# SmoothKen/knn-svc

Hardware: AMD Instinct MI355X
Metric: audio-sec converted/sec (xRT) end-to-end, cold target pool (higher is better)
Workload: dtype f32; 1 GPU; north-star point per rank: 30 s source vs 10 min target pool (20 x 30 s), ckpt_type=mix, post_opt_0.2, cold (pool encoded inside the step); seeded random weights of WavLM-Large (6 layers executed) and the 22.9 M-param generator; nq=1500, np_per_rank=30000, wavlm_batch_chunks=32, pipeline_depth=2

## Files before the change

### knn_svc_amd/csrc/elementwise.hip

```cpp
#include "common.h"
#include <cstdlib>
#include "gemm2_core.h"

namespace {

__device__ __forceinline__ void store_split4(float* row, int c, f32x4 y) {
    g2_u32x2 hi, lo;
    f16x2_split4(y, KN_F16X2_A_SCALE, hi, lo);
    char* ob = (char*)row + (c >> 5) * 128 + (c & 31) * 2;
    *(g2_u32x2*)ob = hi;
    *(g2_u32x2*)(ob + 64) = lo;
}
__device__ __forceinline__ f32x4 load_split4(const float* row, int c) {
    const char* ib = (const char*)row + (c >> 5) * 128 + (c & 31) * 2;
    const g2_u32x2 hi = *(const g2_u32x2*)ib, lo = *(const g2_u32x2*)(ib + 64);
    f32x4 y;
#pragma unroll
    for (int e = 0; e < 4; ++e) {
        const unsigned short hb = (unsigned short)(hi[e >> 1] >> (16 * (e & 1))), lb = (unsigned short)(lo[e >> 1] >> (16 * (e & 1)));
        y[e] = ((float)__builtin_bit_cast(_Float16, hb) + (float)__builtin_bit_cast(_Float16, lb)) * (1.0f / KN_F16X2_A_SCALE);
    }
    return y;
}

__device__ __forceinline__ float gelu_erf(float v) {
#pragma clang fp contract(off)
    return kn_gelu(v);
}

template <int MAXV, int R>
__global__ __launch_bounds__(256) void layernorm_kernel(const float* __restrict__ x, long rows, int dim, int ldx,
                                                       const float* __restrict__ gamma, const float* __restrict__ beta,
                                                       int gelu, float* __restrict__ out, int ldo) {
#pragma clang fp contract(off)
    const int lane = threadIdx.x & 63;
    const long row0 = ((long)blockIdx.x * 4 + (threadIdx.x >> 6)) * R;
    if (row0 >= rows) return;
    f32x4 v[R][MAXV];
    float s[R];
#pragma unroll
    for (int r = 0; r < R; ++r) {
        s[r] = 0.f;
        const bool ok = row0 + r < rows;
        const float* xr = x + (row0 + r) * (long)ldx;
#pragma unroll
        for (int i = 0; i < MAXV; ++i) {
            const int c = lane * 4 + 256 * i;
            if (ok && c < dim) { v[r][i] = *(const f32x4*)(xr + c); s[r] += (v[r][i][0] + v[r][i][1]) + (v[r][i][2] + v[r][i][3]); }
            else v[r][i] = (f32x4){0.f, 0.f, 0.f, 0.f};
        }
    }
    float mean[R], q[R];
#pragma unroll
    for (int r = 0; r < R; ++r) mean[r] = wave_sum(s[r]) / (float)dim;
#pragma unroll
    for (int r = 0; r < R; ++r) {
        q[r] = 0.f;
#pragma unroll
        for (int i = 0; i < MAXV; ++i) {
            const int c = lane * 4 + 256 * i;
            if (c < dim) {
#pragma unroll
                for (int e = 0; e < 4; ++e) { const float d = v[r][i][e] - mean[r]; q[r] = fmaf(d, d, q[r]); }
            }
        }
    }
#pragma unroll
    for (int r = 0; r < R; ++r) {
        const float var = wave_sum(q[r]) / (float)dim;
        const float rstd = 1.0f / sqrtf(var + 1e-5f);
        if (row0 + r >= rows) continue;
        float* orow = out + (row0 + r) * (long)ldo;
#pragma unroll
        for (int i = 0; i < MAXV; ++i) {
            const int c = lane * 4 + 256 * i;
            if (c < dim) {
                const f32x4 g = *(const f32x4*)(gamma + c), b = *(const f32x4*)(beta + c);
                f32x4 y;
#pragma unroll
                for (int e = 0; e < 4; ++e) {
                    float t = fmaf((v[r][i][e] - mean[r]) * rstd, g[e], b[e]);
                    y[e] = (gelu & 1) ? gelu_erf(t) : t;
                }
                if (gelu & 2) store_split4(orow, c, y);
                else *(f32x4*)(orow + c) = y;
            }
        }
    }
}

template <int CPL, int KMAXT, int RP>
__global__ __launch_bounds__(256) void conv0_ln_gelu_kernel(const float* __restrict__ x, long L, long T, int k, int stride,
                                                           const float* __restrict__ w, const float* __restrict__ gamma,
                                                           const float* __restrict__ beta, float* __restrict__ out, int split, int subs) {
    __shared__ float xs[2][64 * 8 + 32];
    const int lane = threadIdx.x & 63, wave = threadIdx.x >> 6;
    const int C = CPL * 64;
    const long b = blockIdx.y;
    const float* xb = x + b * L;
    const int span = 63 * stride + k;
    constexpr int NP = (CPL + 1) / 2;
    f32x2 wr[NP][KMAXT], g[NP], be[NP];
#pragma unroll
    for (int c = 0; c < NP; ++c) {
        const int ch = lane * CPL + 2 * c, ch1 = CPL > 1 ? ch + 1 : ch;
        g[c] = (f32x2){gamma[ch], gamma[ch1]}; be[c] = (f32x2){beta[ch], beta[ch1]};
#pragma unroll
        for (int t = 0; t < KMAXT; ++t) wr[c][t] = t < k ? (f32x2){w[ch * k + t], w[ch1 * k + t]} : (f32x2){0.f, 0.f};
    }
  for (int sub = 0; sub < subs; ++sub) {
    const long m0 = ((long)blockIdx.x * subs + sub) * 64;
    if (m0 >= T) break;
    float* xsb = xs[sub & 1];
    for (int i = threadIdx.x; i < span; i += 256) {
        const long p = m0 * stride + i;
        xsb[i] = p < L ? xb[p] : 0.f;
    }
    __syncthreads();
    for (int r = 0; r < 16; r += RP) {
        f32x2 y[RP][NP];
        float s[RP], mean[RP], q[RP], rstd[RP];
#pragma unroll
        for (int u = 0; u < RP; ++u) {
            const int lm = wave * 16 + r + u;
            float xv[KMAXT];
#pragma unroll
            for (int t = 0; t < KMAXT; ++t) xv[t] = t < k ? xsb[lm * stride + t] : 0.f;
            s[u] = 0.f;
#pragma unroll
            for (int c = 0; c < NP; ++c) {
                f32x2 a = {0.f, 0.f};
#pragma unroll
                for (int t = 0; t < KMAXT; ++t) a = __builtin_elementwise_fma(wr[c][t], (f32x2)(xv[t]), a);
                y[u][c] = a; s[u] += a[0]; if (CPL > 1) s[u] += a[1];
            }
        }
#pragma unroll
        for (int u = 0; u < RP; ++u) mean[u] = (RP > 1 ? wave_sum_dpp(s[u]) : wave_sum(s[u])) / (float)C;
#pragma unroll
        for (int u = 0; u < RP; ++u) {
            q[u] = 0.f;
#pragma unroll
            for (int c = 0; c < CPL; ++c) { const float d = y[u][c >> 1][c & 1] - mean[u]; q[u] += d * d; }
        }
#pragma unroll
        for (int u = 0; u < RP; ++u) rstd[u] = 1.0f / sqrtf((RP > 1 ? wave_sum_dpp(q[u]) : wave_sum(q[u])) / (float)C + 1e-5f);
#pragma unroll
        for (int u = 0; u < RP; ++u) {
            const long m = m0 + wave * 16 + r + u;
            if (m >= T) break;
            float* o = out + (b * T + m) * C + lane * CPL;
#pragma unroll
            for (int c = 0; c < NP; ++c) y[u][c] = kn_gelu2(__builtin_elementwise_fma((y[u][c] - mean[u]) * rstd[u], g[c], be[c]));
            if (CPL % 4 == 0) {
                if (split) {
                    float* orow = out + (b * T + m) * C;
#pragma unroll
                    for (int c = 0; c < CPL; c += 4) store_split4(orow, lane * CPL + c, (f32x4){y[u][c / 2][0], y[u][c / 2][1], y[u][c / 2 + 1][0], y[u][c / 2 + 1][1]});
                } else {
#pragma unroll
                    for (int c = 0; c < CPL; c += 4) *(f32x4*)(o + c) = (f32x4){y[u][c / 2][0], y[u][c / 2][1], y[u][c / 2 + 1][0], y[u][c / 2 + 1][1]};
                }
            } else {
#pragma unroll
                for (int c = 0; c < CPL; ++c) o[c] = y[u][c >> 1][c & 1];
            }
        }
    }
  }
}

__global__ __launch_bounds__(256) void gate_kernel(const float* __restrict__ xn, long rows, int heads, int ldx,
                                                  const float* __restrict__ w2, const float* __restrict__ b2,
                                                  const float* __restrict__ grep_a, float* __restrict__ gate, int split) {
    const int lane = threadIdx.x & 63;
    const long row = (long)blockIdx.x * 4 + (threadIdx.x >> 6);
    if (row >= rows) return;
    const int h = lane >> 2, part = lane & 3;
    float sa = 0.f, sb = 0.f;
    if (h < heads) {
        const float* xr = xn + row * (long)ldx + lane * 16;
#pragma unroll
        for (int e = 0; e < 16; e += 4) {
            const f32x4 xv = split ? load_split4(xn + row * (long)ldx, lane * 16 + e) : *(const f32x4*)(xr + e);
            const f32x4 wa = *(const f32x4*)(w2 + part * 16 + e), wb = *(const f32x4*)(w2 + 64 + part * 16 + e);
#pragma unroll
            for (int t = 0; t < 4; ++t) { sa += xv[t] * wa[t]; sb += xv[t] * wb[t]; }
        }
    }
    sa += __shfl_xor(sa, 1, 64); sa += __shfl_xor(sa, 2, 64);
    sb += __shfl_xor(sb, 1, 64); sb += __shfl_xor(sb, 2, 64);
    if (h < heads && part == 0) {
        const float ga = 1.0f / (1.0f + expf(-(sa + b2[0])));
        const float gb = 1.0f / (1.0f + expf(-(sb + b2[1])));
        gate[row * heads + h] = ga * (gb * grep_a[h] - 1.0f) + 2.0f;
    }
}

__global__ __launch_bounds__(256) void weighted_gather_kernel(const long* __restrict__ idx, const float* __restrict__ w,
                                                             long nq, int k, const float* __restrict__ pool, int dim,
                                                             int ld, float* __restrict__ out) {
#pragma clang fp contract(off)
    const long row = blockIdx.x;
    for (int c = threadIdx.x; c < dim; c += 256) {
        float acc = 0.f;
        for (int j = 0; j < k; ++j) {
            const float wj = w ? w[row * k + j] : 1.0f / (float)k;
            const float t = pool[idx[row * k + j] * (long)ld + c] * wj;
            acc = j == 0 ? t : acc + t;
        }
        out[row * (long)dim + c] = acc;
    }
}

__global__ void reflect_pad_kernel(const float* __restrict__ x, long n, int pad, float* __restrict__ out) {
    const long i = (long)blockIdx.x * blockDim.x + threadIdx.x;
    if (i >= n + 2 * (long)pad) return;
    long j = i - pad;
    if (j < 0) j = -j;
    if (j >= n) j = 2 * (n - 1) - j;
    out[i] = x[j];
}

__global__ void complex_mag_kernel(const float* __restrict__ reim, long rows, int bins, int ld, float* __restrict__ out) {
    const long i = (long)blockIdx.x * blockDim.x + threadIdx.x;
    if (i >= rows * bins) return;
    const long r = i / bins; const int b = (int)(i - r * bins);
    out[i] = hypotf(reim[r * ld + b], reim[r * ld + bins + b]);
}

__global__ void harmonic_amps_kernel(const float* __restrict__ spec, const float* __restrict__ f0, long T, int bins,
                                     int n_harm, float* __restrict__ harm) {
#pragma clang fp contract(off)
    const long i = (long)blockIdx.x * blockDim.x + threadIdx.x;
    if (i >= T * n_harm) return;
    const long t = i / n_harm; const int k = (int)(i - t * n_harm) + 1;
    const float f = f0[t];
    const float* s = spec + t * bins;
    float v;
    if (f == 0.f) {
        if (k == 1) { v = s[0]; for (int b = 1; b < bins; ++b) v = fmaxf(v, s[b]); }
        else v = 0.f;
    } else {
        const int nb = bins * 8;
        float pos = ((f * (float)k) * 2.0f) * (float)nb / 16000.0f;
        pos = fminf(pos, (float)nb);
        const int gi = (int)rintf(pos);
        if (gi >= nb) v = 0.f;
        else {
            float src = ((float)gi + 0.5f) * 0.125f - 0.5f;
            if (src < 0.f) src = 0.f;
            const int i0 = (int)src;
            const int i1 = i0 + (i0 < bins - 1 ? 1 : 0);
            const float l1 = src - (float)i0, l0 = 1.0f - l1;
            v = l0 * s[i0] + l1 * s[i1];
        }
    }
    harm[i] = 0.0108f * v;
}

__global__ __launch_bounds__(256) void reflect_pad_batch_kernel(const float* __restrict__ x, const long* __restrict__ offs, int pad,
                                                                float* __restrict__ out, long stride) {
    const int b = blockIdx.y;
    const long o0 = offs[b], n = offs[b + 1] - o0;
    float* ob = out + (long)b * stride;
    for (long i = (long)blockIdx.x * blockDim.x + threadIdx.x; i < stride; i += (long)gridDim.x * blockDim.x) {
        float v = 0.f;
        if (i < n + 2 * (long)pad) {
            long j = i - pad;
            if (j < 0) j = -j;
            if (j >= n) j = 2 * (n - 1) - j;
            v = x[o0 + j];
        }
        ob[i] = v;
    }
}

__global__ __launch_bounds__(256) void spec_harm_kernel(const float* __restrict__ reim, long rows, int bins, int ld,
                                                        const float* __restrict__ f0, int n_harm, float* __restrict__ spec,
                                                        float* __restrict__ harm) {
#pragma clang fp contract(off)
    extern __shared__ float sh[];
    const int wave = threadIdx.x >> 6, lane = threadIdx.x & 63;
    const long t = (long)blockIdx.x * 4 + wave;
    if (t >= rows) return;
    float* s = sh + wave * bins;
    const float* r = reim + t * (long)ld;
    float mx = 0.f;
    for (int b = lane; b < bins; b += 64) {
        const float v = hypotf(r[b], r[bins + b]);
        s[b] = v; spec[t * bins + b] = v;
        mx = fmaxf(mx, v);
    }
#pragma unroll
    for (int o = 32; o > 0; o >>= 1) mx = fmaxf(mx, __shfl_xor(mx, o, 64));
    const float f = f0[t];
    for (int k = lane + 1; k <= n_harm; k += 64) {
        float v;
        if (f == 0.f) v = k == 1 ? mx : 0.f;
        else {
            const int nb = bins * 8;
            float pos = ((f * (float)k) * 2.0f) * (float)nb / 16000.0f;
            pos = fminf(pos, (float)nb);
            const int gi = (int)rintf(pos);
            if (gi >= nb) v = 0.f;
            else {
                float src = ((float)gi + 0.5f) * 0.125f - 0.5f;
                if (src < 0.f) src = 0.f;
                const int i0 = (int)src;
                const int i1 = i0 + (i0 < bins - 1 ? 1 : 0);
                const float l1 = src - (float)i0, l0 = 1.0f - l1;
                v = l0 * s[i0] + l1 * s[i1];
            }
        }
        harm[t * n_harm + (k - 1)] = 0.0108f * v;
    }
}

__global__ __launch_bounds__(256) void mask_rows_kernel(float* __restrict__ x, int T, int dim, int ld, const int* __restrict__ lens) {
    const int b = blockIdx.y;
    const int len = lens[b];
    const long n4 = (long)(T - len) * (dim / 4);
    for (long i = (long)blockIdx.x * blockDim.x + threadIdx.x; i < n4; i += (long)gridDim.x * blockDim.x) {
        const long r = len + i / (dim / 4); const int c = (int)(i % (dim / 4)) * 4;
        *(f32x4*)(x + ((long)b * T + r) * ld + c) = (f32x4){0.f, 0.f, 0.f, 0.f};
    }
}

}

extern "C" int knnsvc_mask_rows(float* x, int32_t batches, int32_t T, int32_t dim, int32_t ld, const int32_t* lens, void* stream) {
    KN_REQUIRE(x && lens && batches > 0 && batches <= 65535 && T > 0 && dim > 0 && dim % 4 == 0 && ld >= dim && ld % 4 == 0 &&
               ((uintptr_t)x & 15) == 0, "mask_rows: bad arguments");
    hipLaunchKernelGGL(mask_rows_kernel, dim3(64, (unsigned)batches), dim3(256), 0, (hipStream_t)stream, x, T, dim, ld, lens);
    return knnsvc_check_launch("mask_rows");
}

extern "C" int knnsvc_layernorm(const float* x, int64_t rows, int32_t dim, int32_t ldx, const float* gamma,
                                const float* beta, int32_t gelu, float* out, int32_t ldo, void* stream) {
    KN_REQUIRE(x && gamma && beta && out, "layernorm: null pointer");
    KN_REQUIRE(dim > 0 && dim % 4 == 0 && dim <= 2048, "layernorm: dim must be a multiple of 4 and <= 2048");
    KN_REQUIRE(ldx % 4 == 0 && ldo % 4 == 0 && ldx >= dim && ldo >= dim, "layernorm: bad row strides");
    KN_REQUIRE(!(gelu & 2) || (dim % 32 == 0 && ldo % 32 == 0), "layernorm: split output needs dim % 32 == 0 and ldo % 32 == 0");
    KN_REQUIRE(((uintptr_t)x & 15) == 0 && ((uintptr_t)out & 15) == 0 && ((uintptr_t)gamma & 15) == 0 &&
               ((uintptr_t)beta & 15) == 0, "layernorm: pointers must be 16-byte aligned");
    if (rows <= 0) return KNNSVC_OK;
    hipStream_t st = (hipStream_t)stream;
    if (dim <= 512)
        hipLaunchKernelGGL((layernorm_kernel<2, 4>), dim3((unsigned)cdiv64(rows, 16)), dim3(256), 0, st, x, (long)rows, dim, ldx,
                           gamma, beta, gelu, out, ldo);
    else if (dim <= 1024)
        hipLaunchKernelGGL((layernorm_kernel<4, 2>), dim3((unsigned)cdiv64(rows, 8)), dim3(256), 0, st, x, (long)rows, dim, ldx,
                           gamma, beta, gelu, out, ldo);
    else
        hipLaunchKernelGGL((layernorm_kernel<8, 1>), dim3((unsigned)cdiv64(rows, 4)), dim3(256), 0, st, x, (long)rows, dim, ldx,
                           gamma, beta, gelu, out, ldo);
    return knnsvc_check_launch("layernorm");
}

extern "C" int knnsvc_wavlm_gate(const float* xn, int64_t rows, int32_t heads, int32_t head_dim, int32_t ldx,
                                 const float* w2, const float* b2, const float* grep_a, float* gate, int32_t x_f16x2, void* stream) {
    KN_REQUIRE(xn && w2 && b2 && grep_a && gate, "wavlm_gate: null pointer");
    KN_REQUIRE(head_dim == 64 && heads >= 1 && heads <= 16, "wavlm_gate: head_dim must be 64, heads <= 16");
    KN_REQUIRE(ldx % 4 == 0 && ldx >= heads * 64 && ((uintptr_t)xn & 15) == 0 && ((uintptr_t)w2 & 15) == 0,
               "wavlm_gate: alignment");
    if (rows <= 0) return KNNSVC_OK;
    hipLaunchKernelGGL(gate_kernel, dim3((unsigned)cdiv64(rows, 4)), dim3(256), 0, (hipStream_t)stream,
                       xn, (long)rows, heads, ldx, w2, b2, grep_a, gate, x_f16x2);
    return knnsvc_check_launch("wavlm_gate");
}

extern "C" int knnsvc_weighted_gather(const int64_t* idx, const float* w, int64_t nq, int32_t k, const float* pool,
                                      int32_t dim, int32_t ld, int32_t mean_mode, float* out, void* stream) {
    (void)mean_mode;
    KN_REQUIRE(idx && pool && out && k > 0 && dim > 0 && ld >= dim, "weighted_gather: bad arguments");
    KN_REQUIRE(w || (k & (k - 1)) == 0, "weighted_gather: uniform weights need a power-of-two k");
    if (nq <= 0) return KNNSVC_OK;
    hipLaunchKernelGGL(weighted_gather_kernel, dim3((unsigned)nq), dim3(256), 0, (hipStream_t)stream,
                       (const long*)idx, w, (long)nq, k, pool, dim, ld, out);
    return knnsvc_check_launch("weighted_gather");
}

extern "C" int knnsvc_reflect_pad(const float* x, int64_t n, int32_t pad, float* out, void* stream) {
    KN_REQUIRE(x && out && n > pad && pad >= 0, "reflect_pad: needs n > pad >= 0");
    const long tot = n + 2 * (long)pad;
    hipLaunchKernelGGL(reflect_pad_kernel, dim3((unsigned)cdiv64(tot, 256)), dim3(256), 0, (hipStream_t)stream,
                       x, (long)n, pad, out);
    return knnsvc_check_launch("reflect_pad");
}

extern "C" int knnsvc_reflect_pad_batch(const float* x, const int64_t* offs, int32_t batches, int32_t pad, float* out,
                                        int64_t stride, void* stream) {
    KN_REQUIRE(x && offs && out && batches > 0 && batches <= 65535 && pad >= 0 && stride > 2 * (int64_t)pad,
               "reflect_pad_batch: bad arguments (every item needs n > pad; stride > 2 pad)");
    const unsigned gx = (unsigned)(cdiv64(stride, 256) < 2048 ? cdiv64(stride, 256) : 2048);
    hipLaunchKernelGGL(reflect_pad_batch_kernel, dim3(gx, (unsigned)batches), dim3(256), 0, (hipStream_t)stream,
                       x, (const long*)offs, pad, out, (long)stride);
    return knnsvc_check_launch("reflect_pad_batch");
}

extern "C" int knnsvc_spec_harm(const float* reim, int64_t rows, int32_t bins, int32_t ld, const float* f0, int32_t n_harm,
                                float* spec, float* harm, void* stream) {
    KN_REQUIRE(reim && f0 && spec && harm && bins > 0 && bins <= 4096 && ld >= 2 * bins && n_harm > 0, "spec_harm: bad arguments");
    if (rows <= 0) return KNNSVC_OK;
    hipLaunchKernelGGL(spec_harm_kernel, dim3((unsigned)cdiv64(rows, 4)), dim3(256), (size_t)4 * bins * sizeof(float),
                       (hipStream_t)stream, reim, (long)rows, bins, ld, f0, n_harm, spec, harm);
    return knnsvc_check_launch("spec_harm");
}

extern "C" int knnsvc_complex_mag(const float* reim, int64_t rows, int32_t bins, int32_t ld, float* out, void* stream) {
    KN_REQUIRE(reim && out && bins > 0 && ld >= 2 * bins, "complex_mag: bad arguments");
    if (rows <= 0) return KNNSVC_OK;
    hipLaunchKernelGGL(complex_mag_kernel, dim3((unsigned)cdiv64(rows * bins, 256)), dim3(256), 0,
                       (hipStream_t)stream, reim, (long)rows, bins, ld, out);
    return knnsvc_check_launch("complex_mag");
}

extern "C" int knnsvc_harmonic_amps(const float* spec, const float* f0, int64_t T, int32_t bins, int32_t n_harm,
                                    float* harm, void* stream) {
    KN_REQUIRE(spec && f0 && harm && bins > 0 && n_harm > 0, "harmonic_amps: bad arguments");
    if (T <= 0) return KNNSVC_OK;
    hipLaunchKernelGGL(harmonic_amps_kernel, dim3((unsigned)cdiv64(T * n_harm, 256)), dim3(256), 0,
                       (hipStream_t)stream, spec, f0, (long)T, bins, n_harm, harm);
    return knnsvc_check_launch("harmonic_amps");
}

extern "C" int knnsvc_wavlm_conv0(const float* x, int32_t batches, int64_t L, const float* w, int32_t channels, int32_t k,
                                  int32_t stride, const float* gamma, const float* beta, float* out, int32_t out_f16x2, void* stream) {
    KN_REQUIRE(x && w && gamma && beta && out, "wavlm_conv0: null pointer");
    KN_REQUIRE(batches > 0 && batches <= 65535 && L >= k && k >= 1 && k <= 16 && stride >= 1 && stride <= 8,
               "wavlm_conv0: needs 1 <= k <= 16, 1 <= stride <= 8");
    KN_REQUIRE(channels == 64 || channels == 128 || channels == 256 || channels == 512, "wavlm_conv0: channels must be 64/128/256/512");
    KN_REQUIRE(!out_f16x2 || channels >= 256, "wavlm_conv0: split output needs >= 256 channels");
    const long T = (L - k) / stride + 1;
    hipStream_t st = (hipStream_t)stream;
    static int rp = -1, subs_env = -1;
    if (rp < 0) { const char* e = getenv("KNNSVC_CONV0_RP"); rp = e ? atoi(e) : 2; if (rp != 1 && rp != 4) rp = 2; }
    if (subs_env < 0) { const char* e = getenv("KNNSVC_CONV0_SUBS"); subs_env = e ? atoi(e) : 8; if (subs_env < 1 || subs_env > 64) subs_env = 8; }
    const int subs = cdiv64(T, 64L * subs_env) * batches >= 3072 ? subs_env : 1;
    dim3 grid((unsigned)cdiv64(T, 64L * subs), (unsigned)batches);
#define KN_C0R(CPL, KM, RP) hipLaunchKernelGGL((conv0_ln_gelu_kernel<CPL, KM, RP>), grid, dim3(256), 0, st, x, (long)L, T, k, stride, w, gamma, beta, out, out_f16x2, subs)
#define KN_C0(CPL, KM) { if (rp == 2) KN_C0R(CPL, KM, 2); else if (rp == 4) KN_C0R(CPL, KM, 4); else KN_C0R(CPL, KM, 1); }
    if (k <= 10) {
        if (channels == 512) KN_C0(8, 10) else if (channels == 256) KN_C0(4, 10) else if (channels == 128) KN_C0(2, 10) else KN_C0(1, 10)
    } else {
        if (channels == 512) KN_C0(8, 16) else if (channels == 256) KN_C0(4, 16) else if (channels == 128) KN_C0(2, 16) else KN_C0(1, 16)
    }
#undef KN_C0R
#undef KN_C0
    return knnsvc_check_launch("wavlm_conv0");
}

namespace {

__global__ __launch_bounds__(256) void round_f16_kernel(const float* __restrict__ x, long n, float* __restrict__ out) {
    const long i = ((long)blockIdx.x * 256 + threadIdx.x) * 4;
    if (i + 3 < n) {
        const f32x4 v = *(const f32x4*)(x + i);
        f32x4 r;
#pragma unroll
        for (int e = 0; e < 4; ++e) r[e] = (float)(_Float16)v[e];
        *(f32x4*)(out + i) = r;
    } else {
        for (long j = i; j < n; ++j) out[j] = (float)(_Float16)x[j];
    }
}

__global__ __launch_bounds__(256) void amp_ratio_kernel(const float* __restrict__ spec_q, int ld_q,
                                                       const float* __restrict__ spec_pool, int ld_pool, long np,
                                                       const long* __restrict__ idx, long nq, int k, int bins,
                                                       float* __restrict__ out) {
    const int lane = threadIdx.x & 63;
    const long t = (long)blockIdx.x * 4 + (threadIdx.x >> 6);
    if (t >= nq) return;
    double s = 0.0;
    for (int c = lane; c < bins; c += 64) s += (double)fabsf(spec_q[t * ld_q + c]);
    const float orig = (float)wave_sum_d(s);
    for (int j = 0; j < k; ++j) {
        long id = idx[t * k + j];
        id = id < 0 ? 0 : (id > np - 1 ? np - 1 : id);
        double a = 0.0;
        for (int c = lane; c < bins; c += 64) a += (double)fabsf(spec_pool[id * ld_pool + c]);
        const float l1 = (float)wave_sum_d(a);
        if (lane == 0) out[t * k + j] = orig / (l1 + 1e-5f);
    }
}

}

extern "C" int knnsvc_round_f16(const float* x, int64_t n, float* out, void* stream) {
    KN_REQUIRE(x && out && n >= 0, "round_f16: bad arguments");
    KN_REQUIRE(((uintptr_t)x & 15) == 0 && ((uintptr_t)out & 15) == 0, "round_f16: pointers must be 16-byte aligned");
    if (n == 0) return KNNSVC_OK;
    hipLaunchKernelGGL(round_f16_kernel, dim3((unsigned)cdiv64(n, 1024)), dim3(256), 0, (hipStream_t)stream, x, (long)n, out);
    return knnsvc_check_launch("round_f16");
}

extern "C" int knnsvc_amp_ratio(const float* spec_q, int32_t ld_q, const float* spec_pool, int32_t ld_pool, int64_t np,
                                const int64_t* idx, int64_t nq, int32_t k, int32_t bins, float* out, void* stream) {
    KN_REQUIRE(spec_q && spec_pool && idx && out, "amp_ratio: null pointer");
    KN_REQUIRE(np > 0 && k > 0 && bins > 0 && ld_q >= bins && ld_pool >= bins, "amp_ratio: bad sizes");
    if (nq <= 0) return KNNSVC_OK;
    hipLaunchKernelGGL(amp_ratio_kernel, dim3((unsigned)cdiv64(nq, 4)), dim3(256), 0, (hipStream_t)stream, spec_q, ld_q,
                       spec_pool, ld_pool, (long)np, (const long*)idx, (long)nq, k, bins, out);
    return knnsvc_check_launch("amp_ratio");
}
```

Baseline: 918.8 x real-time.

## Compute WavLM conv0 with split-f16 MFMA fused with LayerNorm and GELU

Adds a 512-channel conv0 kernel that runs the first feature-extractor convolution as 16x16x32 f16 MFMA products. Weights and input windows are split into hi/lo f16 pairs with per-block exponent scaling, and three MFMAs per tile recover near-f32 accuracy. LayerNorm and GELU are fused over the accumulators using cross-lane shuffles. It becomes the default for 512 channels, replacing scalar FMA convolution; the old path stays reachable through an env var, and the RP knob is fixed at 2. Risks are extra split and rescale work and small precision differences.

Measured after the change: 925.4 x real-time (median of 6 runs). Within noise of the previous version (+0.7%).

```diff
diff --git a/knn_svc_amd/csrc/elementwise.hip b/knn_svc_amd/csrc/elementwise.hip
--- a/knn_svc_amd/csrc/elementwise.hip
+++ b/knn_svc_amd/csrc/elementwise.hip
@@ -164,6 +164,148 @@
             } else {
 #pragma unroll
                 for (int c = 0; c < CPL; ++c) o[c] = y[u][c >> 1][c & 1];
+            }
+        }
+    }
+  }
+}
+
+template <bool SPLIT>
+__global__ __launch_bounds__(256) void conv0_ln_gelu_mfma_kernel(const float* __restrict__ x, long L, long T, int k, int stride,
+                                                                const float* __restrict__ w, const float* __restrict__ gamma,
+                                                                const float* __restrict__ beta, float* __restrict__ out, int subs) {
+#pragma clang fp contract(off)
+    constexpr int C = 512, NT = C / 16;
+    __shared__ g2_u32x4 wl[NT * 2 * 32];
+    __shared__ f32x4 gl[C / 4], bl[C / 4];
+    __shared__ float xs[2][64 * 8 + 32];
+    __shared__ float wmax[4];
+    const int lane = threadIdx.x & 63, wave = threadIdx.x >> 6;
+    const long b = blockIdx.y;
+    const float* xb = x + b * L;
+    const int span = 63 * stride + k;
+    auto chan0 = [](int i, int q) { return 32 * (i >> 1) + 8 * q + 4 * (i & 1); };
+    float wv[4][8];
+    float am = 0.f;
+#pragma unroll
+    for (int j = 0; j < 4; ++j) {
+        const int p = threadIdx.x + 256 * j, ch = chan0(p >> 5, (p >> 2) & 3) + (p & 3), t0 = ((p >> 4) & 1) * 8;
+#pragma unroll
+        for (int t = 0; t < 8; ++t) { wv[j][t] = t0 + t < k ? w[ch * k + t0 + t] : 0.f; am = fmaxf(am, fabsf(wv[j][t])); }
+    }
+    am = wave_max(am);
+    if (lane == 0) wmax[wave] = am;
+    if (threadIdx.x < C / 4) { gl[threadIdx.x] = *(const f32x4*)(gamma + 4 * threadIdx.x); bl[threadIdx.x] = *(const f32x4*)(beta + 4 * threadIdx.x); }
+    __syncthreads();
+    am = fmaxf(fmaxf(wmax[0], wmax[1]), fmaxf(wmax[2], wmax[3]));
+    int ew = (int)(__builtin_bit_cast(unsigned, am) >> 23);
+    ew = ew < 14 ? 14 : ew > 254 ? 254 : ew;
+    const float w_scale = __builtin_bit_cast(float, (unsigned)(267 - ew) << 23), w_inv = __builtin_bit_cast(float, (unsigned)(ew - 13) << 23);
+#pragma unroll
+    for (int j = 0; j < 4; ++j) {
+        const int p = threadIdx.x + 256 * j;
+        g2_u32x2 h0, l0, h1, l1;
+        f16x2_split4((f32x4){wv[j][0], wv[j][1], wv[j][2], wv[j][3]}, w_scale, h0, l0);
+        f16x2_split4((f32x4){wv[j][4], wv[j][5], wv[j][6], wv[j][7]}, w_scale, h1, l1);
+        wl[((p >> 5) * 2 + 0) * 32 + (p & 31)] = (g2_u32x4){h0[0], h0[1], h1[0], h1[1]};
+        wl[((p >> 5) * 2 + 1) * 32 + (p & 31)] = (g2_u32x4){l0[0], l0[1], l1[0], l1[1]};
+    }
+    const int n = lane & 15, quad = lane >> 4;
+    float xn[3];
+#pragma unroll
+    for (int j = 0; j < 3; ++j) { const long p = (long)blockIdx.x * subs * 64 * stride + threadIdx.x + 256 * j; xn[j] = p < L ? xb[p] : 0.f; }
+  for (int sub = 0; sub < subs; ++sub) {
+    const long m0 = ((long)blockIdx.x * subs + sub) * 64;
+    if (m0 >= T) break;
+    float* xsb = xs[sub & 1];
+#pragma unroll
+    for (int j = 0; j < 3; ++j) if (threadIdx.x + 256 * j < span) xsb[threadIdx.x + 256 * j] = xn[j];
+    __syncthreads();
+    if (sub + 1 < subs) {
+#pragma unroll
+        for (int j = 0; j < 3; ++j) { const long p = (m0 + 64) * stride + threadIdx.x + 256 * j; xn[j] = p < L ? xb[p] : 0.f; }
+    }
+    const int lm = wave * 16 + n;
+    float xv[16], xm = 0.f;
+#pragma unroll
+    for (int t = 0; t < 16; ++t) { xv[t] = t < k ? xsb[lm * stride + t] : 0.f; xm = fmaxf(xm, fabsf(xv[t])); }
+    int ex = (int)(__builtin_bit_cast(unsigned, xm) >> 23);
+    ex = ex < 14 ? 14 : ex > 254 ? 254 : ex;
+    const float x_scale = quad < 2 ? __builtin_bit_cast(float, (unsigned)(267 - ex) << 23) : 0.f;
+    const float t_inv = w_inv * __builtin_bit_cast(float, (unsigned)(ex - 13) << 23);
+    f16x8 xh, xl;
+    {
+        const bool up = quad & 1;
+        g2_u32x2 h0, l0, h1, l1;
+        f16x2_split4((f32x4){up ? xv[8] : xv[0], up ? xv[9] : xv[1], up ? xv[10] : xv[2], up ? xv[11] : xv[3]}, x_scale, h0, l0);
+        f16x2_split4((f32x4){up ? xv[12] : xv[4], up ? xv[13] : xv[5], up ? xv[14] : xv[6], up ? xv[15] : xv[7]}, x_scale, h1, l1);
+        xh = __builtin_bit_cast(f16x8, (g2_u32x4){h0[0], h0[1], h1[0], h1[1]});
+        xl = __builtin_bit_cast(f16x8, (g2_u32x4){l0[0], l0[1], l1[0], l1[1]});
+    }
+    f32x4 acc[NT];
+#pragma unroll
+    for (int i = 0; i < NT; ++i) {
+        const f16x8 wh = __builtin_bit_cast(f16x8, wl[(i * 2 + 0) * 32 + (lane & 31)]), wlo = __builtin_bit_cast(f16x8, wl[(i * 2 + 1) * 32 + (lane & 31)]);
+        f32x4 c = {0.f, 0.f, 0.f, 0.f};
+#ifndef KN_CONV0_WHATIF_NOMFMA
+        c = __builtin_amdgcn_mfma_f32_16x16x32_f16(wlo, xh, c, 0, 0, 0);
+        c = __builtin_amdgcn_mfma_f32_16x16x32_f16(wh, xl, c, 0, 0, 0);
+        c = __builtin_amdgcn_mfma_f32_16x16x32_f16(wh, xh, c, 0, 0, 0);
+#else
+        c[0] = (float)wlo[0] * (float)xh[0]; c[1] = (float)wh[1] * (float)xl[1]; c[2] = (float)wh[2] * (float)xh[2]; c[3] = (float)wh[3];
+#endif
+        acc[i] = c;
+    }
+    f32x4 s4 = {0.f, 0.f, 0.f, 0.f};
+#pragma unroll
+    for (int i = 0; i < NT; ++i) s4 += acc[i];
+    float s = (s4[0] + s4[1]) + (s4[2] + s4[3]);
+    s += __shfl_xor(s, 16, 64);
+    s += __shfl_xor(s, 32, 64);
+    const float mean = s * (1.0f / C);
+    f32x4 q4 = {0.f, 0.f, 0.f, 0.f};
+#pragma unroll
+    for (int i = 0; i < NT; ++i) { const f32x4 d = acc[i] - mean; q4 = __builtin_elementwise_fma(d, d, q4); }
+    float q = (q4[0] + q4[1]) + (q4[2] + q4[3]);
+    q += __shfl_xor(q, 16, 64);
+    q += __shfl_xor(q, 32, 64);
+    const float var = ((q * (1.0f / C)) * t_inv) * t_inv;
+    const float rs = t_inv * (1.0f / sqrtf(var + 1e-5f));
+    const long m = m0 + lm;
+    if (m < T) {
+        float* orow = out + (b * T + m) * C;
+#pragma unroll
+        for (int i = 0; i < NT; i += 2) {
+            f32x4 y[2];
+#pragma unroll
+            for (int u = 0; u < 2; ++u) {
+                const int c0 = chan0(i + u, quad);
+                const f32x4 g = gl[c0 >> 2], be = bl[c0 >> 2];
+                const f32x4 d = (acc[i + u] - mean) * rs;
+#ifndef KN_CONV0_WHATIF_NOGELU
+                const f32x2 y0 = kn_gelu2(__builtin_elementwise_fma((f32x2){d[0], d[1]}, (f32x2){g[0], g[1]}, (f32x2){be[0], be[1]}));
+                const f32x2 y1 = kn_gelu2(__builtin_elementwise_fma((f32x2){d[2], d[3]}, (f32x2){g[2], g[3]}, (f32x2){be[2], be[3]}));
+#else
+                const f32x2 y0 = __builtin_elementwise_fma((f32x2){d[0], d[1]}, (f32x2){g[0], g[1]}, (f32x2){be[0], be[1]});
+                const f32x2 y1 = __builtin_elementwise_fma((f32x2){d[2], d[3]}, (f32x2){g[2], g[3]}, (f32x2){be[2], be[3]});
+#endif
+                y[u] = (f32x4){y0[0], y0[1], y1[0], y1[1]};
+            }
+#ifdef KN_CONV0_WHATIF_NOSTORE
+            if (i == NT - 2 || y[0][0] == 1234.5f || y[1][0] == 1234.5f)
+#endif
+            {
+                if (SPLIT) {
+                    g2_u32x2 h0, l0, h1, l1;
+                    f16x2_split4(y[0], KN_F16X2_A_SCALE, h0, l0);
+                    f16x2_split4(y[1], KN_F16X2_A_SCALE, h1, l1);
+                    char* ob = (char*)orow + (i >> 1) * 128 + quad * 16;
+                    *(g2_u32x4*)ob = ((g2_u32x4){h0[0], h0[1], h1[0], h1[1]});
+                    *(g2_u32x4*)(ob + 64) = ((g2_u32x4){l0[0], l0[1], l1[0], l1[1]});
+                } else {
+                    *(f32x4*)(orow + chan0(i, quad)) = y[0];
+                    *(f32x4*)(orow + chan0(i + 1, quad)) = y[1];
+                }
             }
         }
     }
@@ -434,19 +576,22 @@
     KN_REQUIRE(!out_f16x2 || channels >= 256, "wavlm_conv0: split output needs >= 256 channels");
     const long T = (L - k) / stride + 1;
     hipStream_t st = (hipStream_t)stream;
-    static int rp = -1, subs_env = -1;
-    if (rp < 0) { const char* e = getenv("KNNSVC_CONV0_RP"); rp = e ? atoi(e) : 2; if (rp != 1 && rp != 4) rp = 2; }
+    static int fma = -1, subs_env = -1;
+    if (fma < 0) { const char* e = getenv("KNNSVC_CONV0"); fma = e && e[0] == 'f'; }
     if (subs_env < 0) { const char* e = getenv("KNNSVC_CONV0_SUBS"); subs_env = e ? atoi(e) : 8; if (subs_env < 1 || subs_env > 64) subs_env = 8; }
     const int subs = cdiv64(T, 64L * subs_env) * batches >= 3072 ? subs_env : 1;
     dim3 grid((unsigned)cdiv64(T, 64L * subs), (unsigned)batches);
-#define KN_C0R(CPL, KM, RP) hipLaunchKernelGGL((conv0_ln_gelu_kernel<CPL, KM, RP>), grid, dim3(256), 0, st, x, (long)L, T, k, stride, w, gamma, beta, out, out_f16x2, subs)
-#define KN_C0(CPL, KM) { if (rp == 2) KN_C0R(CPL, KM, 2); else if (rp == 4) KN_C0R(CPL, KM, 4); else KN_C0R(CPL, KM, 1); }
+    if (channels == 512 && !fma) {
+        if (out_f16x2) hipLaunchKernelGGL(conv0_ln_gelu_mfma_kernel<true>, grid, dim3(256), 0, st, x, (long)L, T, k, stride, w, gamma, beta, out, subs);
+        else hipLaunchKernelGGL(conv0_ln_gelu_mfma_kernel<false>, grid, dim3(256), 0, st, x, (long)L, T, k, stride, w, gamma, beta, out, subs);
+        return knnsvc_check_launch("wavlm_conv0");
+    }
+#define KN_C0(CPL, KM) hipLaunchKernelGGL((conv0_ln_gelu_kernel<CPL, KM, 2>), grid, dim3(256), 0, st, x, (long)L, T, k, stride, w, gamma, beta, out, out_f16x2, subs);
     if (k <= 10) {
         if (channels == 512) KN_C0(8, 10) else if (channels == 256) KN_C0(4, 10) else if (channels == 128) KN_C0(2, 10) else KN_C0(1, 10)
     } else {
         if (channels == 512) KN_C0(8, 16) else if (channels == 256) KN_C0(4, 16) else if (channels == 128) KN_C0(2, 16) else KN_C0(1, 16)
     }
-#undef KN_C0R
 #undef KN_C0
     return knnsvc_check_launch("wavlm_conv0");
 }
```
